# aerius-labs/zksnap-circuits-halo2

Measured on AMD Instinct MI355X. Metric: BN254 G1 MSM Mpoints/sec, higher is better.
Workload: dtype u32x9 (254-bit modular integer, radix 2^29); 1 GPU; BN254 G1 MSM, 2^20 random points/scalars per GPU (BASELINE configs[1]), point-range sharded x1, inputs resident in HBM, bases registered once (prepared fixed-base table, as under ParamsKZG::commit); points_per_gpu=1048576, parallelism=point-range shard x1 + all_gather(96 B) + fold

## Files before the change

### zksnap_circuits_halo2_amd/csrc/msm.hip

```cpp
#include <hip/hip_runtime.h>
#include <atomic>
#include <cstdint>
#include <cstdio>
#include <cstring>
#include <cstdlib>
#include <mutex>
#include "ec_quad.hpp"
#include "fe_inverse.hpp"
#include "zkhip_internal.hpp"

namespace zkhip {

static inline size_t align_up(size_t v, size_t a) { return (v + a - 1) / a * a; }

constexpr int FINE_BITS = 12;
constexpr int MAX_GROUPS = 128;
constexpr int MAX_WIDE_W = 16;
struct win_layout { int c, W, narrow; };
__host__ __device__ __forceinline__ int win_bits(const win_layout& L, int w) { return w < L.W - L.narrow ? L.c : L.c - 1; }
__host__ __device__ __forceinline__ int win_off(const win_layout& L, int w) { const int full = L.W - L.narrow; return w <= full ? w * L.c : full * L.c + (w - full) * (L.c - 1); }
static int msm_narrow_windows(int c, int W) {
  static const bool uniform = getenv("ZKHIP_UNIFORM_WINDOWS") != nullptr;
  if (c <= 16 || uniform) return 0;
  const int narrow = W * c - 256;
  return narrow > 0 && narrow <= W ? narrow : 0;
}
constexpr int MAX_TASK_LEN = 128;
constexpr int TASK_SHIFT = 6;

struct task_t {
  uint32_t bucket, start, len;
};

__device__ __forceinline__ xyzz load_xyzz(const uint32_t* base, size_t idx) {
  const uint4* q = reinterpret_cast<const uint4*>(base + idx * 36);
  uint32_t w[36];
#pragma unroll
  for (int i = 0; i < 9; i++) {
    uint4 v = q[i];
    w[4 * i] = v.x; w[4 * i + 1] = v.y; w[4 * i + 2] = v.z; w[4 * i + 3] = v.w;
  }
  xyzz r;
#pragma unroll
  for (int i = 0; i < 9; i++) { r.X.l[i] = w[i]; r.Y.l[i] = w[9 + i]; r.ZZ.l[i] = w[18 + i]; r.ZZZ.l[i] = w[27 + i]; }
  return r;
}

__device__ __forceinline__ void store_xyzz(uint32_t* base, size_t idx, const xyzz& a) {
  uint32_t w[36];
#pragma unroll
  for (int i = 0; i < 9; i++) { w[i] = a.X.l[i]; w[9 + i] = a.Y.l[i]; w[18 + i] = a.ZZ.l[i]; w[27 + i] = a.ZZZ.l[i]; }
  uint4* q = reinterpret_cast<uint4*>(base + idx * 36);
#pragma unroll
  for (int i = 0; i < 9; i++) q[i] = make_uint4(w[4 * i], w[4 * i + 1], w[4 * i + 2], w[4 * i + 3]);
}

__device__ __forceinline__ xyzz xyzz_shfl_xor(const xyzz& a, int mask) {
  xyzz r;
#pragma unroll
  for (int i = 0; i < NL; i++) {
    r.X.l[i] = (uint32_t)__shfl_xor((int)a.X.l[i], mask, 64);
    r.Y.l[i] = (uint32_t)__shfl_xor((int)a.Y.l[i], mask, 64);
    r.ZZ.l[i] = (uint32_t)__shfl_xor((int)a.ZZ.l[i], mask, 64);
    r.ZZZ.l[i] = (uint32_t)__shfl_xor((int)a.ZZZ.l[i], mask, 64);
  }
  return r;
}

__device__ __forceinline__ fe load_fe9_generic(const uint32_t* p, size_t idx) {
  fe r;
#pragma unroll
  for (int i = 0; i < 9; i++) r.l[i] = p[idx * 9 + i];
  return r;
}
__device__ __forceinline__ void store_fe9_generic(uint32_t* p, size_t idx, const fe& a) {
#pragma unroll
  for (int i = 0; i < 9; i++) p[idx * 9 + i] = a.l[i];
}

template <typename DIGIT>
__global__ void __launch_bounds__(256) k_digits(const uint32_t* __restrict__ scalars, DIGIT* __restrict__ digits,
                                                uint32_t n, uint32_t n_pad, int c, int W, uint32_t K, size_t scalar_stride, int narrow) {
  const size_t idx = (size_t)blockIdx.x * blockDim.x + threadIdx.x;
  if (idx >= (size_t)K * n_pad) return;
  const uint32_t kb = (uint32_t)(idx / n_pad), i = (uint32_t)(idx % n_pad);
  digits += (size_t)kb * n_pad;
  const size_t row = (size_t)K * n_pad;
  if (i >= n) {
    for (int win = 0; win < W; win++) digits[(size_t)win * row + i] = 0;
    return;
  }
  uint32_t w[8];
  load_words(scalars + ((size_t)kb * scalar_stride + i) * 8, w);
  fe c32;
#pragma unroll
  for (int k = 0; k < NL; k++) c32.l[k] = FrParams::FROM_EXT_CANON[k];
  fe s = fe_canon_lt2p<FrParams>(fe_mul<FrParams>(c32, fe_unpack<0>(w)));
  fe_pack(s, w);
  const win_layout lay{c, W, narrow};
  uint32_t carry = 0;
  for (int win = 0; win < W; win++) {
    const int bit = win_off(lay, win), cw = win_bits(lay, win);
    const uint32_t half = 1u << (cw - 1), mask = (1u << cw) - 1;
    uint32_t v = 0;
    if (bit < 256) {
      int wi = bit >> 5, sh = bit & 31;
      uint64_t two = w[wi];
      if (wi + 1 < 8) two |= (uint64_t)w[wi + 1] << 32;
      v = (uint32_t)(two >> sh) & mask;
    }
    v += carry;
    int32_t d;
    if (v >= half) { d = (int32_t)v - (int32_t)(1u << cw); carry = 1; } else { d = (int32_t)v; carry = 0; }
    digits[(size_t)win * row + i] = (DIGIT)d;
  }
}

__global__ void __launch_bounds__(1024) k_digits_wide(const uint32_t* __restrict__ scalars, int32_t* __restrict__ digits, uint32_t n, uint32_t n_pad,
                                                       int c, int W, uint32_t* __restrict__ gcount, int narrow) {
  __shared__ uint32_t cnt[MAX_WIDE_W * MAX_GROUPS];
  for (uint32_t t = threadIdx.x; t < (uint32_t)W * MAX_GROUPS; t += blockDim.x) cnt[t] = 0;
  __syncthreads();
  const win_layout lay{c, W, narrow};
  for (uint32_t i = blockIdx.x * blockDim.x + threadIdx.x; i < n_pad; i += gridDim.x * blockDim.x) {
    if (i >= n) {
      for (int win = 0; win < W; win++) digits[(size_t)win * n_pad + i] = 0;
      continue;
    }
    uint32_t w[8];
    load_words(scalars + (size_t)i * 8, w);
    fe c32;
#pragma unroll
    for (int k = 0; k < NL; k++) c32.l[k] = FrParams::FROM_EXT_CANON[k];
    fe sv = fe_canon_lt2p<FrParams>(fe_mul<FrParams>(c32, fe_unpack<0>(w)));
    fe_pack(sv, w);
    uint32_t carry = 0;
    for (int win = 0; win < W; win++) {
      const int bit = win_off(lay, win), cw = win_bits(lay, win);
      const uint32_t half = 1u << (cw - 1), mask = (1u << cw) - 1;
      uint32_t v = 0;
      if (bit < 256) {
        const int wi = bit >> 5, sh = bit & 31;
        uint64_t two = w[wi];
        if (wi + 1 < 8) two |= (uint64_t)w[wi + 1] << 32;
        v = (uint32_t)(two >> sh) & mask;
      }
      v += carry;
      int32_t d;
      if (v >= half) { d = (int32_t)v - (int32_t)(1u << cw); carry = 1; } else { d = (int32_t)v; carry = 0; }
      digits[(size_t)win * n_pad + i] = d;
      if (d != 0) atomicAdd(&cnt[win * MAX_GROUPS + (((uint32_t)(d < 0 ? -d : d) - 1) >> FINE_BITS)], 1u);
    }
  }
  __syncthreads();
  for (uint32_t t = threadIdx.x; t < (uint32_t)W * MAX_GROUPS; t += blockDim.x)
    if (cnt[t]) atomicAdd(&gcount[t], cnt[t]);
}

namespace glv {
__device__ constexpr uint32_t G1[3] = {0xc7e0b3d7u, 0xd91d232eu, 0x2u};
__device__ constexpr uint32_t G2[5] = {0x391eb18eu, 0x7a7bd9d4u, 0xa773d2cfu, 0x4ccef014u, 0x2u};
// ... 842 lines not shown
    xyzz acc = xyzz_identity();
#pragma unroll 1
    for (uint32_t j = lo + threadIdx.x; j < hi; j += 128) acc = xyzz_add(acc, load_xyzz(partials, t + j));
    acc = workgroup_sum_128(acc, xch);
    if (P == 1) {
      if (threadIdx.x == 0) store_xyzz(buckets, k, acc);
      continue;
    }
    if (threadIdx.x == 0) {
      store_xyzz(partials, t + lo, acc);
      __threadfence();
      is_last = atomicAdd(&heavy_done[i - sl], 1u) == P - 1;
    }
    __syncthreads();
    if (!is_last) continue;
    __threadfence();
    acc = xyzz_identity();
#pragma unroll 1
    for (uint32_t j = threadIdx.x; j < P; j += 128) acc = xyzz_add(acc, load_xyzz(partials, t + j * HEAVY_SLICE));
    acc = workgroup_sum_128(acc, xch);
    if (threadIdx.x == 0) store_xyzz(buckets, k, acc);
  }
}

template <int COMBINE_LANES>
__global__ void __launch_bounds__(128) k_combine_seq(const uint32_t* __restrict__ task_off, uint32_t nbuckets,
                                                     uint32_t* __restrict__ partials, uint32_t* __restrict__ buckets,
                                                     uint32_t seq_parts, uint32_t blocks, const uint32_t* __restrict__ heavy_count,
                                                     const uint2* __restrict__ heavy, uint32_t heavy_cap, uint32_t* __restrict__ heavy_done, uint32_t quad_max) {
  __shared__ __attribute__((aligned(16))) uint32_t xch[64 * 36];
  if (blockIdx.x >= blocks) { combine_heavy_buckets(blockIdx.x - blocks, task_off, partials, buckets, heavy_count, heavy, heavy_cap, heavy_done, xch, quad_max); return; }
  const uint32_t gid = blockIdx.x * blockDim.x + threadIdx.x;
  const uint32_t k = gid / COMBINE_LANES, q = gid % COMBINE_LANES;
  const bool live = k < nbuckets;
  xyzz acc = xyzz_identity();
  uint32_t m = 0;
  if (live) {
    const uint32_t t = task_off[k];
    m = task_off[k + 1] - t;
    const uint32_t left = (m == 1 || m > seq_parts) ? 0u : m;
#pragma unroll 1
    for (uint32_t j = q; j < left; j += COMBINE_LANES) acc = xyzz_add(acc, load_xyzz(partials, t + j));
  }
#pragma unroll 1
  for (int mask = 1; mask < COMBINE_LANES; mask <<= 1) acc = xyzz_add(acc, xyzz_shfl_xor(acc, mask));
  if (live && q == 0 && m != 1 && m <= seq_parts) store_xyzz(buckets, k, acc);
}

template <int COMBINE_LANES>
__global__ void __launch_bounds__(128) k_combine_seq_quad(const uint32_t* __restrict__ task_off, uint32_t nbuckets,
                                                          uint32_t* __restrict__ partials, uint32_t* __restrict__ buckets,
                                                          uint32_t seq_parts, uint32_t blocks, const uint32_t* __restrict__ heavy_count,
                                                          const uint2* __restrict__ heavy, uint32_t heavy_cap, uint32_t* __restrict__ heavy_done, uint32_t quad_max) {
  __shared__ __attribute__((aligned(16))) uint32_t xch[64 * 36];
  if (blockIdx.x >= blocks) { combine_heavy_buckets(blockIdx.x - blocks, task_off, partials, buckets, heavy_count, heavy, heavy_cap, heavy_done, xch, quad_max); return; }
  const uint32_t gid = blockIdx.x * blockDim.x + threadIdx.x;
  const uint32_t q = gid & 3, lane = (gid >> 2) % COMBINE_LANES, k = (gid >> 2) / COMBINE_LANES;
  const bool live = k < nbuckets;
  xyzz acc = xyzz_identity();
  uint32_t m = 0;
  if (live) {
    const uint32_t t = task_off[k];
    m = task_off[k + 1] - t;
    const uint32_t left = (m == 1 || m > seq_parts) ? 0u : m;
#pragma unroll 1
    for (uint32_t j = lane; j < left; j += COMBINE_LANES) acc = xyzz_add_quad(acc, load_xyzz(partials, t + j), q);
  }
#pragma unroll 1
  for (int mask = 1; mask < COMBINE_LANES; mask <<= 1) acc = xyzz_add_quad(acc, xyzz_shfl_xor(acc, 4 * mask), q);
  if (live && lane == 0 && q == 0 && m != 1 && m <= seq_parts) store_xyzz(buckets, k, acc);
}

__global__ void __launch_bounds__(128) k_pyramid_step(const uint32_t* __restrict__ in, uint32_t* __restrict__ out,
                                                      uint32_t N, int s, uint32_t in_stride, uint32_t out_stride) {
  const uint32_t per_win = N / 2 + (uint32_t)s * (N / 4);
  const int win = blockIdx.y;
  const uint32_t* wi = in + (size_t)win * in_stride * 36;
  uint32_t* wo = out + (size_t)win * out_stride * 36;
#pragma unroll 1
  for (uint32_t tid = blockIdx.x * blockDim.x + threadIdx.x; tid < per_win; tid += gridDim.x * blockDim.x) {
    uint32_t ia, ib;
    if (tid < N / 2) {
      ia = 2 * tid; ib = 2 * tid + 1;
    } else {
      uint32_t r = tid - N / 2;
      uint32_t l = r / (N / 4), u = r % (N / 4);
      if ((int)l == s - 1) { ia = 4 * u + 1; ib = 4 * u + 3; }
      else { ia = N + l * (N / 2) + 2 * u; ib = ia + 1; }
    }
    store_xyzz(wo, tid, xyzz_add(load_xyzz(wi, ia), load_xyzz(wi, ib)));
  }
}

__global__ void __launch_bounds__(128) k_pyramid_step_quad(const uint32_t* __restrict__ in, uint32_t* __restrict__ out,
                                                           uint32_t N, int s, uint32_t in_stride, uint32_t out_stride) {
  const uint32_t per_win = N / 2 + (uint32_t)s * (N / 4);
  const uint32_t gid = blockIdx.x * blockDim.x + threadIdx.x;
  const uint32_t tid = gid >> 2, q = gid & 3;
  if (tid >= per_win) return;
  const int win = blockIdx.y;
  const uint32_t* wi = in + (size_t)win * in_stride * 36;
  uint32_t* wo = out + (size_t)win * out_stride * 36;
  uint32_t ia, ib;
  if (tid < N / 2) {
    ia = 2 * tid; ib = 2 * tid + 1;
  } else {
    uint32_t r = tid - N / 2;
    uint32_t l = r / (N / 4), u = r % (N / 4);
    if ((int)l == s - 1) { ia = 4 * u + 1; ib = 4 * u + 3; }
    else { ia = N + l * (N / 2) + 2 * u; ib = ia + 1; }
  }
  const xyzz r = xyzz_add_quad(load_xyzz(wi, ia), load_xyzz(wi, ib), q);
  if (q == 0) store_xyzz(wo, tid, r);
}

__global__ void __launch_bounds__(64) k_window_horner(const uint32_t* __restrict__ in, uint32_t in_stride, int nz,
                                                      uint32_t* __restrict__ winsum, int W) {
  const int gid = blockIdx.x * blockDim.x + threadIdx.x;
  const int win = gid >> 5, lane = gid & 31;
  xyzz acc = xyzz_identity();
  if (win < W) {
    const uint32_t* wi = in + (size_t)win * in_stride * 36;
    int dbl = 0;
    if (lane < nz) { acc = load_xyzz(wi, 2 + lane); dbl = lane; }
    else if (lane == nz) { acc = load_xyzz(wi, 1); dbl = nz; }
    else if (lane == nz + 1) acc = xyzz_add(load_xyzz(wi, 0), load_xyzz(wi, 1));
#pragma unroll 1
    for (int i = 0; i < dbl; i++) acc = xyzz_dbl(acc);
  }
#pragma unroll 1
  for (int mask = 1; mask < 32; mask <<= 1) acc = xyzz_add(acc, xyzz_shfl_xor(acc, mask));
  if (win < W && lane == 0) store_xyzz(winsum, win, acc);
}

__global__ void __launch_bounds__(128) k_window_horner_quad(const uint32_t* __restrict__ in, uint32_t in_stride, int nz,
                                                            uint32_t* __restrict__ winsum, uint32_t* __restrict__ jac_out) {
  __shared__ __attribute__((aligned(16))) uint32_t xch[36];
  const int win = blockIdx.x, term = threadIdx.x >> 2;
  const uint32_t q = threadIdx.x & 3;
  const uint32_t* wi = in + (size_t)win * in_stride * 36;
  xyzz acc = xyzz_identity();
  int dbl = 0;
  if (term < nz) { acc = load_xyzz(wi, 2 + term); dbl = term; }
  else if (term == nz) { acc = load_xyzz(wi, 1); dbl = nz; }
  else if (term == nz + 1) acc = xyzz_add_quad(load_xyzz(wi, 0), load_xyzz(wi, 1), q);
#pragma unroll 1
  for (int i = 0; i < dbl; i++) acc = xyzz_dbl_quad(acc, q);
#pragma unroll 1
  for (int mask = 4; mask < 64; mask <<= 1) acc = xyzz_add_quad(acc, xyzz_shfl_xor(acc, mask), q);
  if (threadIdx.x == 64) store_xyzz(xch, 0, acc);
  __syncthreads();
  if (threadIdx.x < 4) {
    acc = xyzz_add_quad(acc, load_xyzz(xch, 0), q);
    if (q == 0) {
      if (jac_out) store_jacobian(acc, jac_out + (size_t)win * 24);
      else store_xyzz(winsum, win, acc);
    }
  }
}

__global__ void __launch_bounds__(64) k_fold(const uint32_t* __restrict__ winsum, int W, int c, uint32_t* __restrict__ out) {
  if (threadIdx.x >= 4 || blockIdx.x != 0) return;
  const uint32_t q = threadIdx.x;
  xyzz acc = load_xyzz(winsum, W - 1);
  for (int w = W - 2; w >= 0; w--) {
#pragma unroll 1
    for (int i = 0; i < c; i++) acc = xyzz_dbl_quad(acc, q);
    acc = xyzz_add_quad(acc, load_xyzz(winsum, w), q);
  }
  if (q == 0) store_jacobian(acc, out);
}

__global__ void __launch_bounds__(64) k_store_results(const uint32_t* __restrict__ winsum, uint32_t K, uint32_t* __restrict__ out) {
  const uint32_t k = blockIdx.x * blockDim.x + threadIdx.x;
  if (k < K) store_jacobian(load_xyzz(winsum, k), out + (size_t)k * 24);
}

__global__ void __launch_bounds__(64) k_sum_jacobian(const uint32_t* __restrict__ in, int m, uint32_t* __restrict__ out, uint32_t stride) {
  const uint32_t q = threadIdx.x & 3;
  const int grp = threadIdx.x >> 2;
  in += (size_t)blockIdx.x * 24;
  out += (size_t)blockIdx.x * 24;
  xyzz acc = xyzz_identity();
  for (int i = grp; i < m; i += 16) acc = xyzz_add_quad(acc, load_jacobian(in + (size_t)i * stride * 24), q);
#pragma unroll 1
  for (int mask = 4; mask < 64; mask <<= 1) {
    if ((mask >> 2) >= m && mask > 4) break;
    acc = xyzz_add_quad(acc, xyzz_shfl_xor(acc, mask), q);
  }
  if (threadIdx.x == 0) store_jacobian(acc, out);
}

static bool msm_top_window_is_degenerate(int c) {
  const int W = (256 + c - 1) / c, top_bits = 254 - (W - 1) * c;
  return top_bits > 0 && top_bits < 6;
}

static bool msm_glv_enabled() {
  static const bool on = getenv("ZKHIP_NO_GLV") == nullptr;
  return on;
}
static inline int msm_windows(int c, bool glv) {
  if (!glv) return (256 + c - 1) / c;
  return (128 + c - 1) / c + ((c == 2 || c == 4) ? 1 : 0);
}

int msm_pick_window(size_t n) {
  const bool glv = msm_glv_enabled();
  int best = 16;
  double best_cost = 1e300;
  for (int c = 2; c <= 16; c++) {
    const int Wi = msm_windows(c, glv), top_bits = (glv ? 127 : 254) - (Wi - 1) * c;
    if (top_bits > 0 && top_bits < 6) continue;
    const double cost = (double)Wi * (10.0 * (double)(glv ? 2 * n : n) + 28.0 * (double)(1u << (c - 1)));
    if (cost < best_cost) { best_cost = cost; best = c; }
  }
  return best;
}


constexpr int MAX_WINDOW_PREPARED = 20;

int msm_pick_window_prepared(size_t n) {
  const bool large = n >= ((size_t)1 << 20);
  int best = 2;
  double best_cost = 1e300;
  for (int c = 2; c <= MAX_WINDOW_PREPARED; c++) {
    const double W = (256 + c - 1) / c, buckets = (double)(1u << (c - 1));
    if (msm_top_window_is_degenerate(c) && c <= 16) continue;
    if (c > 16 && !large) continue;
    if (c == 17) continue;
    double cost;
    if (!large) cost = W * 10.0 * (double)n + 28.0 * buckets;
    else {
      const double eff = c == 20 ? 1.0 : (c == 19 ? 1.13 : (c == 18 ? 1.06 : 1.07));
      cost = W * (10.0 * eff + 1.0) * (double)n + 39.0 * buckets + 1.1e6 * (double)(c - 2) + 13.0e6;
    }
    if (cost < best_cost) { best_cost = cost; best = c; }
  }
  if (n >= ((size_t)1 << 14) && n < ((size_t)3 << 14)) best = 15;
  if (const char* e = getenv("ZKHIP_MAX_WINDOW")) { int m = atoi(e); if (m >= 2 && best > m) best = m; }
  return best;
}

struct msm_layout {
  uint32_t task_shift;
  size_t max_tasks;
  void* digits;
  uint32_t* stage_ref; uint16_t* stage_fine;
  char* zero_lo; size_t zero_bytes;
  uint32_t *gcounters, *counters, *count, *sorted, *offset, *cursor, *task_off, *bsum1, *bsum2;
  task_t* tasks; uint4* order;
  uint32_t *partials, *pyrA, *pyrB, *winsum;
  uint32_t* endo;
  int combine_lanes;
  uint32_t seq_parts;
  uint2* heavy; uint32_t heavy_cap;
  uint32_t* heavy_done;
  size_t total;
};

static uint32_t msm_task_shift(size_t entries , size_t NB, size_t xyzz_bytes = 144) {
  uint32_t task_shift = TASK_SHIFT;
  static const int knob = [] { const char* e = getenv("ZKHIP_TASK_SHIFT"); return e ? atoi(e) : 0; }();
  if (knob >= 2 && knob <= 7) task_shift = (uint32_t)knob;
  else if ((entries >> 7) >= ((size_t)3 << 16)) task_shift = 7;
  const bool g2 = xyzz_bytes == 288;
  if ((entries >> TASK_SHIFT) < ((size_t)1 << (g2 ? 14 : 17))) {
    const double occ = (double)entries / (double)NB;
    double best = 1e300;
    for (uint32_t sh = 2; sh <= (uint32_t)TASK_SHIFT; sh++) {
      const double L = (double)(1u << sh), parts = occ / L;
      const double est = 5.0 * L + (g2 ? 15.0 : 10.0) * (parts > 1.0 ? parts - 1.0 : 0.0);
      if (est < best) { best = est; task_shift = sh; }
    }
  }
  return task_shift;
}

static bool msm_two_level(int c, bool glv, size_t n_in, bool shared_buckets, size_t K) {
  if (c > 16) return true;
  static const long thr_glv = [] { const char* e = getenv("ZKHIP_GLV_TWO_LEVEL_MIN"); return e ? atol(e) : (1L << 18); }();
  static const long thr_prep = [] { const char* e = getenv("ZKHIP_PREP_TWO_LEVEL_MIN"); return e ? atol(e) : (1L << 16); }();
  if (c != 16 || K != 1) return false;
  if (glv) return thr_glv > 0 && n_in >= (size_t)thr_glv;
  return shared_buckets && thr_prep > 0 && n_in >= (size_t)thr_prep;
}

static msm_layout msm_lay_out(char* base, size_t n_in, size_t K, int c, bool prepared, size_t xyzz_bytes = 144, bool glv = false) {
  msm_layout L;
  const size_t n = glv ? 2 * n_in : n_in;
  const size_t W = (size_t)msm_windows(c, glv), B = (size_t)1 << (c - 1), WB = prepared ? K : W, NB = WB * B;
  const bool wide = msm_two_level(c, glv, n_in, prepared, K);
  const size_t nk = n * K, entries = W * nk;
  const size_t n_pad = (n + 7) & ~(size_t)7;
  L.task_shift = msm_task_shift(entries, NB, xyzz_bytes);
  L.max_tasks = (entries >> L.task_shift) + NB + 1;
  const double parts_avg = (double)entries / (double)NB / (double)(1u << L.task_shift);
  L.combine_lanes = parts_avg <= 2.0 ? 1 : (parts_avg <= 4.0 ? 2 : (parts_avg <= 12.0 ? 4 : 8));
  L.seq_parts = 16u * (uint32_t)L.combine_lanes;
  L.heavy_cap = (uint32_t)(std::min<size_t>(L.max_tasks / (L.seq_parts + 1) + 1, NB) + L.max_tasks / HEAVY_SLICE + 1);
  char* p = base;
  auto carve = [&](size_t bytes) { void* r = p; p += align_up(bytes, 256); return r; };
  L.digits = carve(W * K * n_pad * (wide ? sizeof(int32_t) : sizeof(int16_t)));
  L.stage_ref = wide ? (uint32_t*)carve(entries * sizeof(uint32_t)) : nullptr;
  L.stage_fine = wide ? (uint16_t*)carve(entries * sizeof(uint16_t)) : nullptr;
// ... 51 lines not shown
  if (c > 16 && (!shared_buckets || K != 1)) { set_error("msm: windows above 16 bits need one shared bucket set"); return ZKHIP_EINVAL; }
  if (wide && !shared_buckets && (size_t)W * (B >> FINE_BITS) > (size_t)MAX_GROUPS) { set_error("msm: two-level sort: %d windows x %u groups exceed %d", W, B >> FINE_BITS, MAX_GROUPS); return ZKHIP_EINVAL; }
  if (wide && W > MAX_WIDE_W) { set_error("msm: %d windows of %d bits exceed the wide path's %d", W, c, MAX_WIDE_W); return ZKHIP_EINVAL; }
  const msm_layout lay = msm_lay_out((char*)ws, n_in, K, c, shared_buckets, xyzz_bytes, glv);
  if (ws_bytes < lay.total) { set_error("msm: workspace too small (%zu < %zu bytes)", ws_bytes, lay.total); return ZKHIP_EINVAL; }
  const uint32_t task_shift = lay.task_shift;
  const uint32_t n_pad = (uint32_t)((n + 7) & ~(size_t)7);
  void* const digits = lay.digits;
  uint32_t* const stage_ref = lay.stage_ref;
  uint16_t* const stage_fine = lay.stage_fine;
  uint32_t *const gcounters = lay.gcounters, *const counters = lay.counters, *const count = lay.count, *const sorted = lay.sorted,
           *const offset = lay.offset, *const cursor = lay.cursor, *const task_off = lay.task_off, *const bsum1 = lay.bsum1, *const bsum2 = lay.bsum2;
  task_t* const tasks = lay.tasks;
  uint4* const order = lay.order;

  prof_begin(stream);
  HIPCHK(hipMemsetAsync(lay.zero_lo, 0, lay.zero_bytes, stream));
  const size_t sstride = K > 1 ? scalar_stride : n;
  const size_t nk = n * K, max_tasks = lay.max_tasks;
  (void)nk; (void)max_tasks;
  const unsigned dblocks = (unsigned)(((size_t)K * n_pad + 255) / 256);
  const int narrow = (shared_buckets && !glv) ? msm_narrow_windows(c, W) : 0;
  if (glv && wide) hipLaunchKernelGGL(k_digits_glv<int32_t>, dim3((unsigned)((std::max<size_t>(n_in, 8) + 255) / 256)), dim3(256), 0, stream, d_scalars, (int32_t*)digits, (uint32_t)n_in, n_pad, c, W);
  else if (glv) hipLaunchKernelGGL(k_digits_glv<int16_t>, dim3((unsigned)((std::max<size_t>(n_in, 8) + 255) / 256)), dim3(256), 0, stream, d_scalars, (int16_t*)digits, (uint32_t)n_in, n_pad, c, W);
  else if (wide) {
    static const bool fused_count = getenv("ZKHIP_NO_FUSED_COUNT") == nullptr;
    if (fused_count) {
      static const unsigned wg_knob = [] { const char* e = getenv("ZKHIP_DIGIT_WGS"); const int v = e ? atoi(e) : 0; return v >= 64 && v <= 4096 ? (unsigned)v : 0u; }();
      const unsigned wg_cap = wg_knob ? wg_knob : (n_pad > (1u << 21) ? 1024u : 512u);
      const unsigned wblocks = (unsigned)std::min<size_t>(((size_t)n_pad + 1023) / 1024, wg_cap);
      hipLaunchKernelGGL(k_digits_wide, dim3(wblocks), dim3(1024), 0, stream, d_scalars, (int32_t*)digits, (uint32_t)n, n_pad, c, W, gcounters + 1024, narrow);
    } else {
      hipLaunchKernelGGL(k_digits<int32_t>, dim3(dblocks), dim3(256), 0, stream, d_scalars, (int32_t*)digits, (uint32_t)n, n_pad, c, W, K, sstride, narrow);
    }
  }
  else hipLaunchKernelGGL(k_digits<int16_t>, dim3(dblocks), dim3(256), 0, stream, d_scalars, (int16_t*)digits, (uint32_t)n, n_pad, c, W, K, sstride, 0);
  prof_mark(stream, "digits");
  uint32_t chunks = (uint32_t)((n + 65535) / 65536);
  while (chunks * (uint32_t)W * K < 256 && chunks < (n + 4095) / 4096) chunks *= 2;
  if (chunks == 0) chunks = 1;
  const uint32_t chunk = (uint32_t)((((n + chunks - 1) / chunks) + 7) & ~(size_t)7);
  const size_t lds = wide ? ((size_t)4 << FINE_BITS) : (size_t)B * sizeof(uint32_t);
  static std::once_flag attr_once[64];
  static hipError_t attr_err[64];
  int cur_dev = 0;
  HIPCHK(hipGetDevice(&cur_dev));
  std::call_once(attr_once[cur_dev & 63], [&] {
    hipError_t e = hipFuncSetAttribute((const void*)k_sort_pass<false>, hipFuncAttributeMaxDynamicSharedMemorySize, 128 * 1024);
    if (e == hipSuccess) e = hipFuncSetAttribute((const void*)k_sort_pass<true>, hipFuncAttributeMaxDynamicSharedMemorySize, 128 * 1024);
    if (e == hipSuccess) e = hipFuncSetAttribute((const void*)k_fine_sorted, hipFuncAttributeMaxDynamicSharedMemorySize, (2 * (1 << FINE_BITS) + SORT_CHUNK + SORT_CHUNK / 16) * 4);
    attr_err[cur_dev & 63] = e;
  });
  HIPCHK(attr_err[cur_dev & 63]);
  const uint32_t gstride = (wide && !shared_buckets) ? (B >> FINE_BITS) : 0u;
  const int G = wide ? (int)(gstride ? (uint32_t)W * gstride : (B >> FINE_BITS)) : 1;
  const uint32_t sort_chunk = SORT_CHUNK;
  const uint32_t sort_chunks = (uint32_t)(((size_t)W * n + sort_chunk - 1) / sort_chunk) + (uint32_t)G;
  const uint32_t wb_stride = shared_buckets ? 0u : B;
  if (wide) {
    static const bool fused_count2 = getenv("ZKHIP_NO_FUSED_COUNT") == nullptr;
    if (!fused_count2 || glv)
      hipLaunchKernelGGL(k_coarse_count, dim3(chunks, W), dim3(1024), 0, stream, (const int32_t*)digits, n_pad, chunk, gcounters + 1024, gstride);
    hipLaunchKernelGGL(k_group_offsets, dim3(1), dim3(64), 0, stream, gcounters + 1024, W, G, gcounters + 128, gcounters + 3072, gcounters + 512, sort_chunk);
    static_assert(MAX_GROUPS == 128, "k_coarse_sorted scans two groups per lane of one wavefront");
    hipLaunchKernelGGL(k_coarse_sorted, dim3((n_pad + COARSE_CHUNK - 1) / COARSE_CHUNK, W), dim3(1024), 0, stream, (const int32_t*)digits, n_pad, gcounters + 3072,
                       stage_ref, stage_fine, ref_base, ref_stride, gstride);
    prof_mark(stream, "coarse");
    hipLaunchKernelGGL(k_fine_count, dim3(sort_chunks), dim3(1024), 0, stream, stage_fine, gcounters + 128, gcounters + 512, G, count, sort_chunk);
  } else {
    hipLaunchKernelGGL(k_sort_pass<false>, dim3(chunks, W, K), dim3(1024), lds, stream, (const int16_t*)digits, n_pad, chunk, c, count, (uint32_t*)nullptr, wb_stride, ref_base, ref_stride);
  }
  prof_mark(stream, "count");
  const uint32_t nblk = (NB + SCAN_TILE - 1) / SCAN_TILE;
  const bool scan_single = NB <= SCAN_SINGLE_MAX;
  if (scan_single) {
    hipLaunchKernelGGL(k_scan_single<0>, dim3(1), dim3(1024), 0, stream, count, (uint32_t)NB, counters + 0, offset, cursor, 0u, (uint32_t*)nullptr);
  } else {
    hipLaunchKernelGGL(k_scan_sums2, dim3(nblk), dim3(SCAN_BLOCK), 0, stream, count, NB, bsum1, bsum2, task_shift);
    hipLaunchKernelGGL(k_scan_top2, dim3(1), dim3(SCAN_BLOCK), 0, stream, bsum1, bsum2, nblk, counters + 0, counters + 1);
    hipLaunchKernelGGL(k_scan_apply2, dim3(nblk), dim3(SCAN_BLOCK), 0, stream, count, NB, bsum1, bsum2, counters + 0, counters + 1, offset, cursor, task_off, task_shift);
  }
  prof_mark(stream, "scan");
  if (wide) {
    hipLaunchKernelGGL(k_fine_sorted, dim3(sort_chunks), dim3(1024), (size_t)(2u * (1u << FINE_BITS) + SORT_CHUNK + SORT_CHUNK / 16) * 4, stream, stage_fine, stage_ref,
                       gcounters + 128, gcounters + 512, G, cursor, sorted);
  }
  else hipLaunchKernelGGL(k_sort_pass<true>, dim3(chunks, W, K), dim3(1024), lds, stream, (const int16_t*)digits, n_pad, chunk, c, cursor, sorted, wb_stride, ref_base, ref_stride);
  prof_mark(stream, "scatter");
  static const unsigned task_wg_cap = [] { const char* e = getenv("ZKHIP_TASK_WGS"); const int v = e ? atoi(e) : 0; return v >= 1 && v <= 4096 ? (unsigned)v : 256u; }();
  const unsigned task_blocks = (unsigned)std::min<size_t>((NB + 255) / 256, task_wg_cap);
  if (scan_single) {
    hipLaunchKernelGGL(k_scan_single<1>, dim3(1), dim3(1024), 0, stream, count, (uint32_t)NB, counters + 1, task_off, (uint32_t*)nullptr, task_shift, counters + 192);
    hipLaunchKernelGGL(k_make_tasks, dim3(task_blocks), dim3(256), 0, stream, offset, task_off, NB, tasks, task_shift, counters + 2, (uint32_t*)nullptr, lay.seq_parts,
                       counters + 3, lay.heavy, lay.heavy_cap);
  } else {
    hipLaunchKernelGGL(k_make_tasks, dim3(task_blocks), dim3(256), 0, stream, offset, task_off, NB, tasks, task_shift, counters + 2, counters + 32, lay.seq_parts,
                       counters + 3, lay.heavy, lay.heavy_cap);
    hipLaunchKernelGGL(k_order_offsets, dim3(1), dim3(64), 0, stream, counters + 32, counters + 192);
  }
  hipLaunchKernelGGL(k_make_order, dim3(task_blocks), dim3(256), 0, stream, offset, task_off, NB, task_shift, counters + 192, sorted, order);
  prof_mark(stream, "tasks");
  out->c = c; out->W = W; out->WB = WB; out->B = B; out->NB = NB; out->task_shift = task_shift; out->max_tasks = lay.max_tasks; out->nk = n * K;
  out->tasks = tasks; out->ntasks = counters + 1; out->max_parts = counters + 2; out->order = order; out->sorted = sorted; out->task_off = task_off;
  out->partials = lay.partials; out->pyrA = lay.pyrA; out->pyrB = lay.pyrB; out->winsum = lay.winsum;
  out->combine_lanes = lay.combine_lanes; out->seq_parts = lay.seq_parts; out->heavy_count = counters + 3; out->heavy = lay.heavy; out->heavy_cap = lay.heavy_cap; out->heavy_done = lay.heavy_done;
  out->endo = lay.endo;
  HIPCHK(hipGetLastError());
  return ZKHIP_OK;
}

static int msm_accumulate_combine(const msm_tasks_view& tv, const uint32_t* d_bases, bool prepared, bool glv, size_t n, uint32_t* buckets, hipStream_t stream) {
  const uint32_t NB = tv.NB;
  const size_t max_tasks = tv.max_tasks;
  const task_t* const tasks = (const task_t*)tv.tasks;
  uint32_t* const counters = tv.ntasks - 1;
  const uint4* const order = tv.order;
  const uint32_t *const sorted = tv.sorted, *const task_off = tv.task_off;
  uint32_t* const partials = tv.partials;
  {
    uint32_t blocks = (uint32_t)((max_tasks + 127) / 128);
    if (blocks > 256 * 64) blocks = 256 * 64;
    if (prepared) hipLaunchKernelGGL(k_accumulate<true>, dim3(blocks), dim3(128), 0, stream, tasks, counters + 1, order, sorted, d_bases, partials, buckets, (const uint32_t*)nullptr, 0xffffffffu);
    else hipLaunchKernelGGL(k_accumulate<false>, dim3(blocks), dim3(128), 0, stream, tasks, counters + 1, order, sorted, d_bases, partials, buckets, (const uint32_t*)tv.endo,
                            glv ? (uint32_t)n : 0xffffffffu);
  }
  prof_mark(stream, "accumulate");
  {
    const int combine_lanes = tv.combine_lanes;
    const uint32_t seq_parts = tv.seq_parts;
    const size_t lanes_total = (size_t)NB * combine_lanes;
    const bool quad = lanes_total * 4 <= 131072;
    static const uint32_t heavy_quad_max = [] { const char* e = getenv("ZKHIP_HEAVY_QUAD_MAX"); const long v = e ? atol(e) : -1; return v >= 0 && v <= 2048 ? (uint32_t)v : HEAVY_QUAD_MAX; }();
    const unsigned blocks = (unsigned)((lanes_total * (quad ? 4 : 1) + 127) / 128);
#define ZK_LAUNCH_COMBINE(L)                                                                                                                        \
    do {                                                                                                                                              \
      if (quad) hipLaunchKernelGGL(k_combine_seq_quad<L>, dim3(blocks + HEAVY_WGS), dim3(128), 0, stream, task_off, NB, partials, buckets, seq_parts, blocks,   \
                                   tv.heavy_count, (const uint2*)tv.heavy, tv.heavy_cap, tv.heavy_done, heavy_quad_max);                              \
      else hipLaunchKernelGGL(k_combine_seq<L>, dim3(blocks + HEAVY_WGS), dim3(128), 0, stream, task_off, NB, partials, buckets, seq_parts, blocks,             \
                              tv.heavy_count, (const uint2*)tv.heavy, tv.heavy_cap, tv.heavy_done, heavy_quad_max);                                   \
    } while (0)
    if (combine_lanes == 1) ZK_LAUNCH_COMBINE(1);
    else if (combine_lanes == 2) ZK_LAUNCH_COMBINE(2);
    else if (combine_lanes == 4) ZK_LAUNCH_COMBINE(4);
    else ZK_LAUNCH_COMBINE(8);
#undef ZK_LAUNCH_COMBINE
  }
  prof_mark(stream, "combine");
  return ZKHIP_OK;
}

static int msm_reduce_buckets(int WB, uint32_t B, int c, uint32_t K, bool prepared, uint32_t* cur, uint32_t* nxt, uint32_t* winsum, uint32_t* d_out, hipStream_t stream) {
  static const size_t quad_max = [] { const char* e = getenv("ZKHIP_PYR_QUAD_MAX"); const long v = e ? atol(e) : 0; return v >= 256 && v <= (1 << 20) ? (size_t)v : (size_t)65536; }();
  static const long pyr_persist = [] { const char* e = getenv("ZKHIP_PYR_PERSIST"); const long v = e ? atol(e) : 0; return v >= 64 && v <= 65536 ? v : 0L; }();
  uint32_t in_stride = B;
  int nz = 0;
  {
    uint32_t N = B;
    int s = 1;
    while (N > 2) {
      uint32_t per_win = N / 2 + (uint32_t)s * (N / 4);
      uint32_t out_stride = per_win;
      if ((size_t)per_win * WB <= quad_max) hipLaunchKernelGGL(k_pyramid_step_quad, dim3((4 * per_win + 127) / 128, WB), dim3(128), 0, stream, cur, nxt, N, s, in_stride, out_stride);
      else {
        unsigned blocks = (per_win + 127) / 128;
        if (pyr_persist > 0 && WB == 1) blocks = std::min<unsigned>(blocks, (unsigned)pyr_persist);
        hipLaunchKernelGGL(k_pyramid_step, dim3(blocks, WB), dim3(128), 0, stream, cur, nxt, N, s, in_stride, out_stride);
      }
      uint32_t* t = cur; cur = nxt; nxt = t;
      in_stride = out_stride;
      N >>= 1;
      s++;
    }
    nz = s - 1;
  }
  prof_mark(stream, "pyramid");
  if (B == 1) { set_error("msm: internal: B == 1"); return ZKHIP_EINVAL; }
  const bool direct = prepared && WB <= 2048;
  if (WB <= 2048) hipLaunchKernelGGL(k_window_horner_quad, dim3(WB), dim3(128), 0, stream, cur, in_stride, nz, winsum, direct ? d_out : (uint32_t*)nullptr);
  else hipLaunchKernelGGL(k_window_horner, dim3((WB * 32 + 63) / 64), dim3(64), 0, stream, cur, in_stride, nz, winsum, WB);
  prof_mark(stream, "horner");
  if (prepared) { if (!direct) hipLaunchKernelGGL(k_store_results, dim3((K + 63) / 64), dim3(64), 0, stream, winsum, K, d_out); }
  else hipLaunchKernelGGL(k_fold, dim3(1), dim3(64), 0, stream, winsum, WB, c, d_out);
  prof_mark(stream, "fold");
  HIPCHK(hipGetLastError());
  return ZKHIP_OK;
}

int msm_g1_device(const uint32_t* d_scalars, const uint32_t* d_bases, size_t n, uint32_t* d_out, void* ws, size_t ws_bytes,
                  int c_override, hipStream_t stream, const prepared_bases* prepared, size_t prepared_off, size_t batch,
                  size_t scalar_stride) {
  if (batch == 0) return ZKHIP_OK;
  if (n == 0) {
    for (size_t k = 0; k < batch; k++) hipLaunchKernelGGL(k_sum_jacobian, dim3(1), dim3(64), 0, stream, (const uint32_t*)nullptr, 0, d_out + k * 24, 1u);
    HIPCHK(hipGetLastError());
    return ZKHIP_OK;
  }
  if (batch > 1 && (!prepared || prepared->c > 16 || batch > 65535)) { set_error("msm: batch needs prepared bases with a window <= 16 bits"); return ZKHIP_EINVAL; }
  const uint32_t K = (uint32_t)batch;
  if (n >= (1ull << 31)) { set_error("msm: n = %zu too large", n); return ZKHIP_EINVAL; }
  const int c = prepared ? prepared->c : (c_override > 0 ? c_override : msm_pick_window(n));
  if (c < 2 || c > (prepared ? MAX_WINDOW_PREPARED : 16)) { set_error("msm: window bits %d out of range", c); return ZKHIP_EINVAL; }
  if (prepared) {
    if (prepared_off + n > prepared->n) { set_error("msm: range exceeds the prepared bases"); return ZKHIP_EINVAL; }
    if ((size_t)((256 + c - 1) / c) * prepared->n >= (1ull << 31)) { set_error("msm: prepared table too large for 31-bit point references"); return ZKHIP_EINVAL; }
    d_bases = prepared->table;
    if (prepared->direct && batch == 1) return msm_g1_direct(d_scalars, n, prepared, prepared_off, d_out, ws, ws_bytes, stream);
  }
  msm_tasks_view tv;
  const bool glv = msm_uses_glv(prepared != nullptr, batch, 144);
  int rc = msm_build_tasks(d_scalars, n, batch, scalar_stride, c, prepared != nullptr, prepared ? (uint32_t)prepared_off : 0u, prepared ? (uint32_t)prepared->n : 0u,
                           144, ws, ws_bytes, stream, &tv, glv);
  if (rc != ZKHIP_OK) return rc;
  if (glv) hipLaunchKernelGGL(k_endo_bases, dim3((unsigned)((n + 255) / 256)), dim3(256), 0, stream, d_bases, (uint32_t)n, tv.endo);
  if ((rc = msm_accumulate_combine(tv, d_bases, prepared != nullptr, glv, n, tv.pyrA, stream)) != ZKHIP_OK) return rc;
  return msm_reduce_buckets(tv.WB, tv.B, c, K, prepared != nullptr, tv.pyrA, tv.pyrB, tv.winsum, d_out, stream);
}

__global__ void __launch_bounds__(128) k_bucket_sets_add(uint32_t* __restrict__ acc, const uint32_t* __restrict__ add, uint32_t nb) {
  const uint32_t k = blockIdx.x * blockDim.x + threadIdx.x;
  if (k >= nb) return;
  store_xyzz(acc, k, xyzz_add(load_xyzz(acc, k), load_xyzz(add, k)));
}

static size_t msm_chunk_lay_bytes(size_t chunk_cap, int c) {
  size_t b = msm_lay_out(nullptr, chunk_cap, 1, c, true).total;
  if (chunk_cap > 1) b = std::max(b, msm_lay_out(nullptr, chunk_cap - 1, 1, c, true).total);
  return align_up(b, 256);
}

size_t msm_chunk_workspace_bytes(size_t chunk_cap, int c) {
  if (chunk_cap == 0) return 0;
  return msm_chunk_lay_bytes(chunk_cap, c) + align_up(((size_t)1 << (c - 1)) * 144, 256);
}

int msm_chunk_add(const uint32_t* d_scalars, size_t n, const prepared_bases* pb, size_t pb_off, size_t chunk_cap, bool first, void* ws, size_t ws_bytes, hipStream_t stream) {
  if (!pb || n == 0 || n > chunk_cap || pb_off + n > pb->n) { set_error("msm_chunk_add: bad piece (n = %zu, capacity %zu)", n, chunk_cap); return ZKHIP_EINVAL; }
  const size_t lay_bytes = msm_chunk_lay_bytes(chunk_cap, pb->c);
  if (ws_bytes < msm_chunk_workspace_bytes(chunk_cap, pb->c)) { set_error("msm_chunk_add: workspace too small"); return ZKHIP_EINVAL; }
  uint32_t* const acc = (uint32_t*)((char*)ws + lay_bytes);
  msm_tasks_view tv;
  int rc = msm_build_tasks(d_scalars, n, 1, 0, pb->c, true, (uint32_t)pb_off, (uint32_t)pb->n, 144, ws, lay_bytes, stream, &tv, false);
  if (rc != ZKHIP_OK) return rc;
  if ((rc = msm_accumulate_combine(tv, pb->table, true, false, n, first ? acc : tv.pyrA, stream)) != ZKHIP_OK) return rc;
  if (!first) hipLaunchKernelGGL(k_bucket_sets_add, dim3((tv.NB + 127) / 128), dim3(128), 0, stream, acc, (const uint32_t*)tv.pyrA, tv.NB);
  HIPCHK(hipGetLastError());
  return ZKHIP_OK;
}

int msm_chunk_finish(const prepared_bases* pb, size_t chunk_cap, uint32_t* d_out, void* ws, size_t ws_bytes, hipStream_t stream) {
  if (!pb || ws_bytes < msm_chunk_workspace_bytes(chunk_cap, pb->c)) { set_error("msm_chunk_finish: workspace too small"); return ZKHIP_EINVAL; }
  const msm_layout lay = msm_lay_out((char*)ws, chunk_cap, 1, pb->c, true);
  uint32_t* const acc = (uint32_t*)((char*)ws + msm_chunk_lay_bytes(chunk_cap, pb->c));
  return msm_reduce_buckets(1, 1u << (pb->c - 1), pb->c, 1, true, acc, lay.pyrA, lay.winsum, d_out, stream);
}


constexpr int GEN_CHUNK = 32;

__device__ __forceinline__ xyzz scalar_mul_affine(const uint32_t (&kw)[8], const fe& gx, const fe& gy) {
  xyzz acc = xyzz_identity();
  for (int bit = 255; bit >= 0; bit--) {
    acc = xyzz_dbl(acc);
    if ((kw[bit >> 5] >> (bit & 31)) & 1) xyzz_madd(acc, gx, gy);
  }
  return acc;
}

__device__ __forceinline__ fe fq_inverse(const fe& a) { return fe_inverse<Fq>(a); }

__global__ void __launch_bounds__(64) k_gen_walk(const uint32_t* __restrict__ t0_d ,
                                                 uint32_t n, uint32_t* __restrict__ out, uint32_t* __restrict__ tmp_pts,
                                                 uint32_t* __restrict__ tmp_pref) {
  const uint32_t j = blockIdx.x * blockDim.x + threadIdx.x;
  const uint32_t lo = j * GEN_CHUNK;
  if (lo >= n) return;
  const uint32_t cnt = min((uint32_t)GEN_CHUNK, n - lo);
  uint32_t w0[8], wd[8], kw[8];
#pragma unroll
  for (int i = 0; i < 8; i++) { w0[i] = t0_d[i]; wd[i] = t0_d[8 + i]; }
  fe one_r = fe_one<FrParams>();
  fe t0 = fe_mul<FrParams>(one_r, fe_from_ext_lazy(w0));
  fe dd = fe_mul<FrParams>(one_r, fe_from_ext_lazy(wd));
  fe lo_f = fe_zero();
  lo_f.l[0] = lo & LMASK; lo_f.l[1] = lo >> LB;
  fe r2; 
#pragma unroll
  for (int i = 0; i < NL; i++) r2.l[i] = FrParams::R2[i];
  fe lo_m = fe_mul<FrParams>(r2, lo_f);
  fe k = fe_norm(fe_add(t0, fe_mul<FrParams>(lo_m, dd)));
  fe raw1;
#pragma unroll
  for (int i = 0; i < NL; i++) raw1.l[i] = FrParams::RAW_ONE[i];
  fe kc = fe_canon_lt2p<FrParams>(fe_mul<FrParams>(raw1, k));
  fe_pack(kc, kw);
  fe dc = fe_canon_lt2p<FrParams>(fe_mul<FrParams>(raw1, dd));
  uint32_t dw[8];
  fe_pack(dc, dw);
  fe gx = fe_one<Fq>();
  fe gy = fe_norm(fe_dbl(gx));
  xyzz P = scalar_mul_affine(kw, gx, gy);
  xyzz D = scalar_mul_affine(dw, gx, gy);
  fe pref = fe_one<Fq>();
  for (uint32_t i = 0; i < cnt; i++) {
    store_xyzz(tmp_pts, lo + i, P);
    store_fe9_generic(tmp_pref, lo + i, pref);
    if (!xyzz_is_identity(P)) pref = fe_mul<Fq>(pref, fe_mul<Fq>(P.ZZ, P.ZZZ));
    P = xyzz_add(P, D);
  }
  fe inv = fq_inverse(pref);
  for (uint32_t ii = cnt; ii-- > 0;) {
    xyzz Q = load_xyzz(tmp_pts, lo + ii);
    uint32_t* o = out + (size_t)(lo + ii) * 16;
    if (xyzz_is_identity(Q)) {
#pragma unroll
      for (int t = 0; t < 16; t++) o[t] = 0;
      continue;
    }
    fe pre = load_fe9_generic(tmp_pref, lo + ii);
    fe winv = fe_mul<Fq>(inv, pre);
    inv = fe_mul<Fq>(inv, fe_mul<Fq>(Q.ZZ, Q.ZZZ));
    fe x = fe_mul<Fq>(fe_mul<Fq>(winv, Q.ZZZ), Q.X);
    fe y = fe_mul<Fq>(fe_mul<Fq>(winv, Q.ZZ), Q.Y);
    uint32_t wx[8], wy[8];
    fe_to_ext<Fq>(x, wx);
    fe_to_ext<Fq>(y, wy);
#pragma unroll
    for (int t = 0; t < 8; t++) { o[t] = wx[t]; o[8 + t] = wy[t]; }
  }
}

static void fr_pow2_montgomery(int e, uint32_t out[8]) {
  static const uint64_t RMOD[4] = {0x43e1f593f0000001ull, 0x2833e84879b97091ull, 0xb85045b68181585dull, 0x30644e72e131a029ull};
// ... 593 lines not shown
```

Baseline: 760.6 Mpoints/s.

## Fuse pyramid reduction steps into LDS-resident span kernels with fused Horner close

Replaces the one-launch-per-level pyramid bucket reduction with a planned sequence of span kernels. Each span processes several pyramid levels for a sub-block inside LDS. The final span also performs the window Horner combination in the same kernel. The intent is to cut kernel launch count and the global-memory round trips between levels. In exchange it adds gather/scatter index arithmetic, LDS pressure, and fewer blocks (possibly low occupancy) at small levels, and it is enabled by default.

```diff
diff --git a/zksnap_circuits_halo2_amd/csrc/msm.hip b/zksnap_circuits_halo2_amd/csrc/msm.hip
--- a/zksnap_circuits_halo2_amd/csrc/msm.hip
+++ b/zksnap_circuits_halo2_amd/csrc/msm.hip
@@ -7,6 +7,7 @@
 #include <mutex>
 #include "ec_quad.hpp"
 #include "fe_inverse.hpp"
+#include "pyramid_plan.hpp"
 #include "zkhip_internal.hpp"
 
 namespace zkhip {
@@ -1155,6 +1156,74 @@
   __syncthreads();
   if (threadIdx.x < 4) {
     acc = xyzz_add_quad(acc, load_xyzz(xch, 0), q);
+    if (q == 0) {
+      if (jac_out) store_jacobian(acc, jac_out + (size_t)win * 24);
+      else store_xyzz(winsum, win, acc);
+    }
+  }
+}
+
+template <bool CLOSE>
+__global__ void __launch_bounds__(256) k_pyramid_span(const uint32_t* __restrict__ in, uint32_t* __restrict__ out, uint32_t N, uint32_t M, int s_a, int j,
+                                                      uint32_t in_stride, uint32_t out_stride, uint32_t lds_a, uint32_t single_min,
+                                                      uint32_t* __restrict__ winsum, uint32_t* __restrict__ jac_out) {
+  extern __shared__ __attribute__((aligned(16))) uint32_t pyr_lds[];
+  const uint32_t b = blockIdx.x, q = threadIdx.x & 3;
+  const int win = blockIdx.y;
+  const uint32_t* wi = in + (size_t)win * in_stride * 36;
+  uint32_t* wo = out + (size_t)win * out_stride * 36;
+  uint32_t* const reg_a = pyr_lds + 36;
+  uint32_t* const reg_b = reg_a + (size_t)lds_a * 36;
+  const uint32_t Nout = N >> j;
+#pragma unroll 1
+  for (int i = 0; i < j; i++) {
+    const uint32_t Nl = M >> i;
+    const int s = s_a + i;
+    const uint32_t adds = pyr_level_size(Nl, s);
+    const bool first = i == 0, last = !CLOSE && i == j - 1;
+    const uint32_t* src = first ? wi : (i & 1 ? reg_a : reg_b);
+    uint32_t* dst = last ? wo : (i & 1 ? reg_b : reg_a);
+    if (adds >= single_min) {
+#pragma unroll 1
+      for (uint32_t t = threadIdx.x; t < adds; t += blockDim.x) {
+        pyr_pair p = pyr_level_inputs(Nl, s, t);
+        if (first) { p.a = pyr_span_gather(N, M, b, p.a); p.b = pyr_span_gather(N, M, b, p.b); }
+        store_xyzz(dst, last ? pyr_span_scatter(Nout, b, t) : t, xyzz_add(load_xyzz(src, p.a), load_xyzz(src, p.b)));
+      }
+    } else {
+#pragma unroll 1
+      for (uint32_t t = threadIdx.x >> 2; t < adds; t += blockDim.x >> 2) {
+        pyr_pair p = pyr_level_inputs(Nl, s, t);
+        if (first) { p.a = pyr_span_gather(N, M, b, p.a); p.b = pyr_span_gather(N, M, b, p.b); }
+        const xyzz r = xyzz_add_quad(load_xyzz(src, p.a), load_xyzz(src, p.b), q);
+        if (q == 0) store_xyzz(dst, last ? pyr_span_scatter(Nout, b, t) : t, r);
+      }
+    }
+    __syncthreads();
+  }
+  if (!CLOSE) return;
+  const int nz = s_a + j - 1;
+  if (j == 0) {
+    if (threadIdx.x < (uint32_t)nz + 2) store_xyzz(reg_a, threadIdx.x, load_xyzz(wi, threadIdx.x));
+    __syncthreads();
+  }
+  const uint32_t* fin = (j & 1) || j == 0 ? reg_a : reg_b;
+  xyzz acc = xyzz_identity();
+  if (threadIdx.x < 128) {
+    const int term = threadIdx.x >> 2;
+    int dbl = 0;
+    if (term < nz) { acc = load_xyzz(fin, 2 + term); dbl = term; }
+    else if (term == nz) { acc = load_xyzz(fin, 1); dbl = nz; }
+    else if (term == nz + 1) acc = xyzz_add_quad(load_xyzz(fin, 0), load_xyzz(fin, 1), q);
+#pragma unroll 1
+    for (int i = 0; i < dbl; i++) acc = xyzz_dbl_quad(acc, q);
+#pragma unroll 1
+    for (int mask = 4; mask < 64; mask <<= 1) acc = xyzz_add_quad(acc, xyzz_shfl_xor(acc, mask), q);
+  }
+  if (threadIdx.x == 64) store_xyzz(pyr_lds, 0, acc);
+  __syncthreads();
+  if (threadIdx.x < 4) {
+    acc = xyzz_add_quad(acc, load_xyzz(pyr_lds, 0), q);
     if (q == 0) {
       if (jac_out) store_jacobian(acc, jac_out + (size_t)win * 24);
       else store_xyzz(winsum, win, acc);
@@ -1512,32 +1581,63 @@
 static int msm_reduce_buckets(int WB, uint32_t B, int c, uint32_t K, bool prepared, uint32_t* cur, uint32_t* nxt, uint32_t* winsum, uint32_t* d_out, hipStream_t stream) {
   static const size_t quad_max = [] { const char* e = getenv("ZKHIP_PYR_QUAD_MAX"); const long v = e ? atol(e) : 0; return v >= 256 && v <= (1 << 20) ? (size_t)v : (size_t)65536; }();
   static const long pyr_persist = [] { const char* e = getenv("ZKHIP_PYR_PERSIST"); const long v = e ? atol(e) : 0; return v >= 64 && v <= 65536 ? v : 0L; }();
+  static const bool pyr_fuse = [] { const char* e = getenv("ZKHIP_PYR_FUSE"); return !(e && atoi(e) == 0); }();
+  static const auto pow2_knob = [](const char* name, long lo, long hi, long dflt) { const char* e = getenv(name); const long v = e ? atol(e) : 0; return (uint32_t)(v >= lo && v <= hi && !(v & (v - 1)) ? v : dflt); };
+  static const uint32_t span_block = pow2_knob("ZKHIP_PYR_SPAN_BLOCK", 4, PYR_MAX_BLOCK, PYR_MAX_BLOCK), span_rest = pow2_knob("ZKHIP_PYR_SPAN_REST", 4, PYR_MAX_BLOCK, PYR_REST_BLOCK);
+  static const int span_lead = [] { const char* e = getenv("ZKHIP_PYR_SPAN_LEAD"); const long v = e ? atol(e) : 0; return e && v >= 0 && v <= 18 ? (int)v : -1; }();
+  if (B == 1) { set_error("msm: internal: B == 1"); return ZKHIP_EINVAL; }
+  const bool direct = prepared && WB <= 2048;
   uint32_t in_stride = B;
   int nz = 0;
-  {
+  const auto launch_step = [&](uint32_t N, int s) {
+    const uint32_t per_win = pyr_level_size(N, s);
+    if ((size_t)per_win * WB <= quad_max) hipLaunchKernelGGL(k_pyramid_step_quad, dim3((4 * per_win + 127) / 128, WB), dim3(128), 0, stream, cur, nxt, N, s, in_stride, per_win);
+    else {
+      unsigned blocks = (per_win + 127) / 128;
+      if (pyr_persist > 0 && WB == 1) blocks = std::min<unsigned>(blocks, (unsigned)pyr_persist);
+      hipLaunchKernelGGL(k_pyramid_step, dim3(blocks, WB), dim3(128), 0, stream, cur, nxt, N, s, in_stride, per_win);
+    }
+    uint32_t* t = cur; cur = nxt; nxt = t;
+    in_stride = per_win;
+  };
+  if (pyr_fuse) {
+    const bool close = WB <= 2048;
+    const pyr_plan plan(B, close, span_block, span_lead >= 0 ? span_lead : pyr_lead_steps(B, (uint32_t)WB), span_rest);
+    for (int s = 1; s <= plan.lead; s++) launch_step(B >> (s - 1), s);
+    for (int k = 0; k < plan.count; k++) {
+      const pyr_span& p = plan.span[k];
+      const int j = p.s_b - p.s_a + 1;
+      const uint32_t lds_a = pyr_span_lds_a(p), lds_b = pyr_span_lds_b(p);
+      const size_t lds_bytes = (size_t)(1 + lds_a + lds_b) * 144;
+      if (p.close) {
+        prof_mark(stream, "pyramid");
+        hipLaunchKernelGGL(k_pyramid_span<true>, dim3(1, WB), dim3(256), lds_bytes, stream, cur, nxt, p.N, p.M, p.s_a, j, p.in_stride, p.out_stride, lds_a, PYR_SINGLE_MIN,
+                           winsum, direct ? d_out : (uint32_t*)nullptr);
+      } else {
+        hipLaunchKernelGGL(k_pyramid_span<false>, dim3(p.items, WB), dim3(256), lds_bytes, stream, cur, nxt, p.N, p.M, p.s_a, j, p.in_stride, p.out_stride, lds_a, PYR_SINGLE_MIN,
+                           (uint32_t*)nullptr, (uint32_t*)nullptr);
+        uint32_t* t = cur; cur = nxt; nxt = t;
+      }
+    }
+    in_stride = plan.final_stride;
+    nz = plan.nz;
+    if (!close) {
+      prof_mark(stream, "pyramid");
+      hipLaunchKernelGGL(k_window_horner, dim3((WB * 32 + 63) / 64), dim3(64), 0, stream, cur, in_stride, nz, winsum, WB);
+    }
+  } else {
     uint32_t N = B;
     int s = 1;
     while (N > 2) {
-      uint32_t per_win = N / 2 + (uint32_t)s * (N / 4);
-      uint32_t out_stride = per_win;
-      if ((size_t)per_win * WB <= quad_max) hipLaunchKernelGGL(k_pyramid_step_quad, dim3((4 * per_win + 127) / 128, WB), dim3(128), 0, stream, cur, nxt, N, s, in_stride, out_stride);
-      else {
-        unsigned blocks = (per_win + 127) / 128;
-        if (pyr_persist > 0 && WB == 1) blocks = std::min<unsigned>(blocks, (unsigned)pyr_persist);
-        hipLaunchKernelGGL(k_pyramid_step, dim3(blocks, WB), dim3(128), 0, stream, cur, nxt, N, s, in_stride, out_stride);
-      }
-      uint32_t* t = cur; cur = nxt; nxt = t;
-      in_stride = out_stride;
+      launch_step(N, s);
       N >>= 1;
       s++;
     }
     nz = s - 1;
-  }
-  prof_mark(stream, "pyramid");
-  if (B == 1) { set_error("msm: internal: B == 1"); return ZKHIP_EINVAL; }
-  const bool direct = prepared && WB <= 2048;
-  if (WB <= 2048) hipLaunchKernelGGL(k_window_horner_quad, dim3(WB), dim3(128), 0, stream, cur, in_stride, nz, winsum, direct ? d_out : (uint32_t*)nullptr);
-  else hipLaunchKernelGGL(k_window_horner, dim3((WB * 32 + 63) / 64), dim3(64), 0, stream, cur, in_stride, nz, winsum, WB);
+    prof_mark(stream, "pyramid");
+    if (WB <= 2048) hipLaunchKernelGGL(k_window_horner_quad, dim3(WB), dim3(128), 0, stream, cur, in_stride, nz, winsum, direct ? d_out : (uint32_t*)nullptr);
+    else hipLaunchKernelGGL(k_window_horner, dim3((WB * 32 + 63) / 64), dim3(64), 0, stream, cur, in_stride, nz, winsum, WB);
+  }
   prof_mark(stream, "horner");
   if (prepared) { if (!direct) hipLaunchKernelGGL(k_store_results, dim3((K + 63) / 64), dim3(64), 0, stream, winsum, K, d_out); }
   else hipLaunchKernelGGL(k_fold, dim3(1), dim3(64), 0, stream, winsum, WB, c, d_out);
diff --git a/zksnap_circuits_halo2_amd/csrc/pyramid_plan.hpp b/zksnap_circuits_halo2_amd/csrc/pyramid_plan.hpp
--- /dev/null
+++ b/zksnap_circuits_halo2_amd/csrc/pyramid_plan.hpp
@@ -0,0 +1,105 @@
+#pragma once
+#include <cstdint>
+
+#if defined(__HIPCC__)
+#define ZK_PYR_HD __host__ __device__ inline
+#else
+#define ZK_PYR_HD inline
+#endif
+
+namespace zkhip {
+
+constexpr uint32_t PYR_LDS_POINTS = 448;
+constexpr uint32_t PYR_MAX_BLOCK = 256;
+constexpr uint32_t PYR_REST_BLOCK = 16;
+constexpr uint32_t PYR_WIDE_LEVEL = 65536;
+constexpr uint32_t PYR_SINGLE_MIN = 128;
+constexpr int PYR_MAX_SPANS = 20;
+
+struct pyr_pair { uint32_t a, b; };
+
+ZK_PYR_HD uint32_t pyr_level_size(uint32_t N, int s) { return N / 2 + (uint32_t)s * (N / 4); }
+ZK_PYR_HD uint32_t pyr_state_size(uint32_t N, int s) { return N + (uint32_t)(s - 1) * (N / 2); }
+
+ZK_PYR_HD pyr_pair pyr_level_inputs(uint32_t N, int s, uint32_t t) {
+  pyr_pair p;
+  if (t < N / 2) { p.a = 2 * t; p.b = 2 * t + 1; return p; }
+  const uint32_t r = t - N / 2, l = r / (N / 4), u = r % (N / 4);
+  if ((int)l == s - 1) { p.a = 4 * u + 1; p.b = 4 * u + 3; }
+  else { p.a = N + l * (N / 2) + 2 * u; p.b = p.a + 1; }
+  return p;
+}
+
+ZK_PYR_HD uint32_t pyr_span_gather(uint32_t N, uint32_t M, uint32_t b, uint32_t x) {
+  if (x < M) return b * M + x;
+  const uint32_t l = (x - M) / (M / 2), u = (x - M) % (M / 2);
+  return N + l * (N / 2) + b * (M / 2) + u;
+}
+
+ZK_PYR_HD uint32_t pyr_span_scatter(uint32_t Nout, uint32_t b, uint32_t t) {
+  if (t < 2) return 2 * b + t;
+  return Nout + (t - 2) * (Nout / 2) + b;
+}
+
+ZK_PYR_HD uint32_t pyr_span_block(int s) {
+  uint32_t M = PYR_MAX_BLOCK;
+  while (M > 4 && pyr_level_size(M, s) + pyr_level_size(M / 2, s + 1) > PYR_LDS_POINTS) M >>= 1;
+  return M;
+}
+
+inline int pyr_lead_steps(uint32_t B, uint32_t WB) {
+  int lead = 0;
+  for (uint32_t N = B; N > 4 && (uint64_t)pyr_level_size(N, lead + 1) * WB > PYR_WIDE_LEVEL; N >>= 1) lead++;
+  return lead;
+}
+
+struct pyr_span {
+  int s_a, s_b;
+  uint32_t N;
+  uint32_t M;
+  uint32_t items;
+  uint32_t in_stride;
+  uint32_t out_stride;
+  bool close;
+};
+
+inline uint32_t pyr_span_lds_a(const pyr_span& p) { return p.s_b >= p.s_a ? pyr_level_size(p.M, p.s_a) : 2u; }
+inline uint32_t pyr_span_lds_b(const pyr_span& p) { return p.s_b > p.s_a ? pyr_level_size(p.M / 2, p.s_a + 1) : 0u; }
+
+struct pyr_plan {
+  int lead = 0;
+  int count = 0;
+  pyr_span span[PYR_MAX_SPANS];
+  int nz = 0;
+  uint32_t final_stride = 0;
+  pyr_plan(uint32_t B, bool close, uint32_t first_block = PYR_MAX_BLOCK, int lead_steps = 0, uint32_t rest_block = PYR_MAX_BLOCK) {
+    uint32_t N = B, stride = B;
+    int s = 1;
+    while (lead < lead_steps && N > 4) {
+      N >>= 1; s++; lead++;
+      stride = pyr_state_size(N, s);
+    }
+    while (N > 2 || (close && N == 2)) {
+      pyr_span& p = span[count];
+      uint32_t cap = pyr_span_block(s);
+      const uint32_t want = count == 0 ? first_block : rest_block;
+      if (want < cap) cap = want;
+      count++;
+      p.s_a = s; p.N = N; p.in_stride = stride;
+      p.M = N <= cap ? N : cap;
+      p.close = close && p.M == N;
+      int j = 0;
+      while ((4u << j) <= p.M) j++;
+      p.s_b = s + j - 1;
+      p.items = N / p.M;
+      N >>= j; s += j;
+      stride = pyr_state_size(N, s);
+      p.out_stride = stride;
+      if (p.close) break;
+    }
+    nz = s - 1;
+    final_stride = stride;
+  }
+};
+
+}
```

Result: faster. 770.7 Mpoints/s, median of 6 (+1.3%).
